# pps-lab/rofl-project-code

Measured on AMD Instinct MI355X. Metric: range-proof elements/sec (create+verify), d=25k 32-bit, higher is better.
Workload: dtype u32x8 (255-bit integer field)

## Files before the change

include/rofl_zk_debug.h:

```cpp
#ifndef ROFL_ZK_DEBUG_H
#define ROFL_ZK_DEBUG_H
#include "rofl_zk.h"
#ifdef __cplusplus
extern "C" {
#endif

typedef struct {
    double total_ms;
    double msm_accumulate_ms;
    uint64_t msm_accumulate_launches;
    uint64_t msm_terms;
    double fold_ms;
    uint64_t fold_launches;
    uint64_t fold_point_reads;
    double host_ms;
    uint64_t msm_additions;
} rofl_timing_t;
int rofl_last_timing(rofl_timing_t *out);
enum { ROFL_TK_MSM_ACCUMULATE_FB = 0, ROFL_TK_MSM_ACCUMULATE_GEN = 1, ROFL_TK_MSM_SCATTER = 2, ROFL_TK_MSM_REDUCE = 3,
       ROFL_TK_MSM_SMALL = 4, ROFL_TK_FOLD_TAB = 5, ROFL_TK_FOLD = 6, ROFL_TK_OTHER = 7,
       ROFL_TK_SIGMA = 8,
       ROFL_TK_VERIFY_SCALARS = 9,
       ROFL_TK_CODEC = 10,
       ROFL_TK_COUNT = 11 };
// ... 60 lines not shown
int rofl_dbg_rotate_tile_log2(void);
int rofl_dbg_host_dh(const uint8_t sk32[32], const uint8_t *own_pk32, const uint8_t peer_pk32[32], uint8_t out32[32], uint8_t *status);
int rofl_dbg_host_shamir_share(size_t n_secrets, const uint8_t *secrets32, const uint8_t *coef_seeds32, size_t threshold, size_t n_shares,
                               const uint32_t *xs, uint8_t *shares_out32);
int rofl_dbg_host_shamir_reconstruct(size_t n_secrets, size_t n_shares, const uint32_t *xs, const uint8_t *shares32, uint8_t *secrets_out32);
int rofl_dbg_host_feldman_commit(size_t n_secrets, const uint8_t *secrets32, const uint8_t *coef_seeds32, size_t threshold,
                                 uint8_t *commitments_out32);
int rofl_dbg_host_feldman_verify(size_t n_secrets, size_t threshold, const uint8_t *commitments32, size_t n_shares, const uint32_t *xs,
                                 const uint8_t *shares32, uint8_t *verdict_out);
int rofl_dbg_host_sig_sign(size_t n_keys, const uint8_t *sk32, uint8_t *pk_out32, size_t n_msgs, const uint8_t *msg_bytes,
                           const uint64_t *msg_off, size_t n, const rofl_sig_ref_t *refs, uint8_t *sig_out64);
int rofl_dbg_host_sig_verify(size_t n_keys, const uint8_t *pk32, size_t n_msgs, const uint8_t *msg_bytes, const uint64_t *msg_off,
                             size_t n, const rofl_sig_ref_t *refs, const uint8_t *sig64, uint8_t *verdict_out);
int rofl_dbg_host_aead_seal(size_t n_keys, const uint8_t *key32, const uint64_t *derive_round, size_t n, const uint32_t *key_idx,
                            const uint8_t *nonce12, const uint8_t *ad_bytes, const uint64_t *ad_off, const uint8_t *pt_bytes,
                            const uint64_t *pt_off, uint8_t *sealed_out);
int rofl_dbg_host_aead_open(size_t n_keys, const uint8_t *key32, const uint64_t *derive_round, size_t n, const uint32_t *key_idx,
                            const uint8_t *nonce12, const uint8_t *ad_bytes, const uint64_t *ad_off, const uint8_t *sealed_bytes,
                            const uint64_t *sealed_off, uint8_t *pt_out, uint8_t *verdict_out);
int rofl_dbg_poly1305(size_t n, const uint8_t *key32 , const uint8_t *msg_bytes, const uint64_t *msg_off ,
                      uint8_t *tag_out16 );
int rofl_dbg_host_poly1305(size_t n, const uint8_t *key32, const uint8_t *msg_bytes, const uint64_t *msg_off, uint8_t *tag_out16);
int rofl_dbg_host_dleq_prove(size_t n_own, const uint8_t *sk32, uint8_t *own_pk_out32, size_t n_peer, const uint8_t *peer_pk32, size_t n_pairs,
                             const rofl_dh_pair_t *pairs, const uint8_t *ctx32, uint8_t *reveal_out32, uint8_t *proof_out64, uint8_t *status_out);
int rofl_dbg_host_dleq_verify(size_t n_own, const uint8_t *own_pk32, size_t n_peer, const uint8_t *peer_pk32, size_t n_pairs,
                              const rofl_dh_pair_t *pairs, const uint8_t *ctx32, const uint8_t *reveal32, const uint8_t *proof64,
                              uint8_t *shared_out32, uint8_t *verdict_out);
int rofl_dbg_var_mul2(size_t n, const uint8_t *k1_32, const uint8_t *p1_32, const uint8_t *k2_32, const uint8_t *p2_32, uint8_t *out32, double *kernel_ms);
int rofl_dbg_var_mul_sum(size_t n, const uint8_t *k1_32, const uint8_t *p1_32, const uint8_t *k2_32, const uint8_t *p2_32, uint8_t *out32, double *kernel_ms);
int rofl_dbg_lane_scan(const uint8_t *needle, size_t n, int *found);

int rofl_dbg_host_bench(int what, unsigned iters, double *ns_out);
int rofl_dbg_host_horner8_selftest(unsigned W, unsigned c, int lanes, double *us_simd, double *us_scalar);
int rofl_dbg_host_encode8_selftest(unsigned batches, double *us_simd, double *us_scalar);
int rofl_dbg_host_merlin8_selftest(int lanes, unsigned count, unsigned skew, double *us_simd, double *us_scalar);
int rofl_dbg_host_merlin8_lbl3_selftest(int lanes, unsigned count, unsigned skew, double *us_simd, double *us_scalar);
int rofl_dbg_host_merlin8_lbl3_strided_selftest(int lanes, unsigned count, unsigned skew, unsigned stride, double *us_simd, double *us_scalar);
int rofl_dbg_host_merlin_run_selftest(unsigned count, unsigned skew);
int rofl_dbg_host_keccak_zmm_selftest(unsigned states, unsigned chain, double *ns_zmm, double *ns_scalar);
int rofl_dbg_last_hops(double out[10]);

#ifdef __cplusplus
}
#endif
#endif
```

rofl_project_code_amd/csrc/host51x8.hpp:

```cpp
#pragma once
#include <immintrin.h>
#include <string.h>
#include "host51.hpp"

namespace rofl {
namespace h8 {

#define ROFL_H8 __attribute__((target("avx512f,avx512ifma,avx512dq,avx512vl"))) inline

typedef __m512i V;
struct fe8 { V v[5]; };
struct ge8 { fe8 X, Y, Z, T; };

inline bool available() {
    static const bool ok = __builtin_cpu_supports("avx512f") && __builtin_cpu_supports("avx512ifma") && __builtin_cpu_supports("avx512dq");
    return ok;
}

ROFL_H8 V bc(u64 x) { return _mm512_set1_epi64((long long)x); }
ROFL_H8 void carry(fe8 &h) {
    const V M = bc(h51::M51);
    V c;
    c = _mm512_srli_epi64(h.v[0], 51); h.v[0] = _mm512_and_si512(h.v[0], M); h.v[1] = _mm512_add_epi64(h.v[1], c);
    c = _mm512_srli_epi64(h.v[1], 51); h.v[1] = _mm512_and_si512(h.v[1], M); h.v[2] = _mm512_add_epi64(h.v[2], c);
    c = _mm512_srli_epi64(h.v[2], 51); h.v[2] = _mm512_and_si512(h.v[2], M); h.v[3] = _mm512_add_epi64(h.v[3], c);
    c = _mm512_srli_epi64(h.v[3], 51); h.v[3] = _mm512_and_si512(h.v[3], M); h.v[4] = _mm512_add_epi64(h.v[4], c);
    c = _mm512_srli_epi64(h.v[4], 51); h.v[4] = _mm512_and_si512(h.v[4], M);
    V c19 = _mm512_add_epi64(_mm512_add_epi64(_mm512_slli_epi64(c, 4), _mm512_slli_epi64(c, 1)), c);
    h.v[0] = _mm512_add_epi64(h.v[0], c19);
    c = _mm512_srli_epi64(h.v[0], 51); h.v[0] = _mm512_and_si512(h.v[0], M); h.v[1] = _mm512_add_epi64(h.v[1], c);
}
ROFL_H8 fe8 add(const fe8 &a, const fe8 &b) { fe8 r; for (int i = 0; i < 5; i++) r.v[i] = _mm512_add_epi64(a.v[i], b.v[i]); carry(r); return r; }
ROFL_H8 fe8 sub(const fe8 &a, const fe8 &b) {
    fe8 r;
    r.v[0] = _mm512_sub_epi64(_mm512_add_epi64(a.v[0], bc(0x1fffffffffffb4ULL)), b.v[0]);
    for (int i = 1; i < 5; i++) r.v[i] = _mm512_sub_epi64(_mm512_add_epi64(a.v[i], bc(0x1ffffffffffffcULL)), b.v[i]);
    carry(r); return r;
}
ROFL_H8 fe8 mul(const fe8 &a, const fe8 &b) {
    const V Z = _mm512_setzero_si512();
    V lo[9], hi[9];
    for (int k = 0; k < 9; k++) { lo[k] = Z; hi[k] = Z; }
#pragma GCC unroll 5
    for (int i = 0; i < 5; i++)
#pragma GCC unroll 5
        for (int j = 0; j < 5; j++) {
            lo[i + j] = _mm512_madd52lo_epu64(lo[i + j], a.v[i], b.v[j]);
            hi[i + j] = _mm512_madd52hi_epu64(hi[i + j], a.v[i], b.v[j]);
        }
    V col[10];
    col[0] = lo[0];
    for (int c = 1; c < 9; c++) col[c] = _mm512_add_epi64(lo[c], _mm512_slli_epi64(hi[c - 1], 1));
    col[9] = _mm512_slli_epi64(hi[8], 1);
    fe8 r;
    for (int c = 0; c < 5; c++) {
        V x = col[c + 5];
        V x19 = _mm512_add_epi64(_mm512_add_epi64(_mm512_slli_epi64(x, 4), _mm512_slli_epi64(x, 1)), x);
        r.v[c] = _mm512_add_epi64(col[c], x19);
    }
    carry(r); return r;
}
ROFL_H8 fe8 sq(const fe8 &a) {
    const V Z = _mm512_setzero_si512();
    V lo[9], hi[9], xl[9], xh[9];
    for (int k = 0; k < 9; k++) { lo[k] = Z; hi[k] = Z; xl[k] = Z; xh[k] = Z; }
#pragma GCC unroll 5
    for (int i = 0; i < 5; i++) {
        lo[2 * i] = _mm512_madd52lo_epu64(lo[2 * i], a.v[i], a.v[i]);
        hi[2 * i] = _mm512_madd52hi_epu64(hi[2 * i], a.v[i], a.v[i]);
#pragma GCC unroll 5
        for (int j = i + 1; j < 5; j++) {
            xl[i + j] = _mm512_madd52lo_epu64(xl[i + j], a.v[i], a.v[j]);
            xh[i + j] = _mm512_madd52hi_epu64(xh[i + j], a.v[i], a.v[j]);
        }
    }
    V col[10];
    for (int c = 0; c < 10; c++) {
        V x = c < 9 ? _mm512_add_epi64(lo[c], _mm512_slli_epi64(xl[c], 1)) : Z;
        if (c > 0) x = _mm512_add_epi64(x, _mm512_add_epi64(_mm512_slli_epi64(hi[c - 1], 1), _mm512_slli_epi64(xh[c - 1], 2)));
        col[c] = x;
    }
    fe8 r;
    for (int c = 0; c < 5; c++) {
        V x = col[c + 5];
        V x19 = _mm512_add_epi64(_mm512_add_epi64(_mm512_slli_epi64(x, 4), _mm512_slli_epi64(x, 1)), x);
        r.v[c] = _mm512_add_epi64(col[c], x19);
    }
    carry(r); return r;
}
ROFL_H8 fe8 zero() { fe8 r; for (int i = 0; i < 5; i++) r.v[i] = _mm512_setzero_si512(); return r; }
ROFL_H8 fe8 neg(const fe8 &a) { return sub(zero(), a); }
ROFL_H8 fe8 bcast(const h51::fe5 &a) { fe8 r; for (int i = 0; i < 5; i++) r.v[i] = bc(a.v[i]); return r; }

ROFL_H8 ge8 gadd(const ge8 &p, const ge8 &q, const fe8 &d2) {
    fe8 A = mul(sub(p.Y, p.X), sub(q.Y, q.X)), B = mul(add(p.Y, p.X), add(q.Y, q.X));
    fe8 C = mul(mul(p.T, q.T), d2), D = mul(p.Z, q.Z); D = add(D, D);
    fe8 E = sub(B, A), F = sub(D, C), G = add(D, C), H = add(B, A);
    ge8 r = {mul(E, F), mul(G, H), mul(F, G), mul(E, H)};
    return r;
}
ROFL_H8 ge8 gdouble(const ge8 &p) {
    fe8 A = sq(p.X), B = sq(p.Y), C = sq(p.Z); C = add(C, C);
    fe8 E = sub(sub(sq(add(p.X, p.Y)), A), B), G = sub(B, A), F = sub(G, C), H = neg(add(A, B));
    ge8 r = {mul(E, F), mul(G, H), mul(F, G), mul(E, H)};
    return r;
}

ROFL_H8 ge8 load8(const ge *const pts[8]) {
    alignas(64) u64 t[4][5][8];
    for (int l = 0; l < 8; l++) {
        const fe *co[4] = {&pts[l]->X, &pts[l]->Y, &pts[l]->Z, &pts[l]->T};
        for (int c = 0; c < 4; c++) { h51::fe5 f = h51::from_fe_loose(*co[c]); for (int i = 0; i < 5; i++) t[c][i][l] = f.v[i]; }
    }
    ge8 r; fe8 *dst[4] = {&r.X, &r.Y, &r.Z, &r.T};
    for (int c = 0; c < 4; c++) { for (int i = 0; i < 5; i++) dst[c]->v[i] = _mm512_load_si512((const void *)t[c][i]); carry(*dst[c]); }
    return r;
}
ROFL_H8 void store8(h51::ge5 out[8], const ge8 &p) {
    alignas(64) u64 t[4][5][8];
    const fe8 *src[4] = {&p.X, &p.Y, &p.Z, &p.T};
    for (int c = 0; c < 4; c++) for (int i = 0; i < 5; i++) _mm512_store_si512((void *)t[c][i], src[c]->v[i]);
    for (int l = 0; l < 8; l++) {
        h51::fe5 *dst[4] = {&out[l].X, &out[l].Y, &out[l].Z, &out[l].T};
        for (int c = 0; c < 4; c++) for (int i = 0; i < 5; i++) dst[c]->v[i] = t[c][i][l];
    }
}

template <class GetPt>
ROFL_H8 void horner8(h51::ge5 out[8], int lanes, int W, const u32 *pos, GetPt wsum) {
    const fe8 d2 = bcast(h51::K().d2);
    const ge *p8[8];
    for (int l = 0; l < 8; l++) p8[l] = wsum(l < lanes ? l : 0, W - 1);
    ge8 acc = load8(p8);
    for (int w = W - 2; w >= 0; w--) {
        for (u32 i = pos[w]; i < pos[w + 1]; i++) acc = gdouble(acc);
        for (int l = 0; l < 8; l++) p8[l] = wsum(l < lanes ? l : 0, w);
        acc = gadd(acc, load8(p8), d2);
    }
    store8(out, acc);
}

typedef __mmask8 M8;
ROFL_H8 fe8 freeze(fe8 t) {
    const V M = bc(h51::M51);
    carry(t); carry(t);
    t.v[0] = _mm512_add_epi64(t.v[0], bc(19)); carry(t);
    t.v[0] = _mm512_add_epi64(t.v[0], bc((1ULL << 51) - 19));
    for (int i = 1; i < 5; i++) t.v[i] = _mm512_add_epi64(t.v[i], bc((1ULL << 51) - 1));
    V c;
    c = _mm512_srli_epi64(t.v[0], 51); t.v[0] = _mm512_and_si512(t.v[0], M); t.v[1] = _mm512_add_epi64(t.v[1], c);
    c = _mm512_srli_epi64(t.v[1], 51); t.v[1] = _mm512_and_si512(t.v[1], M); t.v[2] = _mm512_add_epi64(t.v[2], c);
    c = _mm512_srli_epi64(t.v[2], 51); t.v[2] = _mm512_and_si512(t.v[2], M); t.v[3] = _mm512_add_epi64(t.v[3], c);
    c = _mm512_srli_epi64(t.v[3], 51); t.v[3] = _mm512_and_si512(t.v[3], M); t.v[4] = _mm512_add_epi64(t.v[4], c);
    t.v[4] = _mm512_and_si512(t.v[4], M);
    return t;
}
ROFL_H8 M8 isneg(const fe8 &a) { fe8 c = freeze(a); return _mm512_test_epi64_mask(c.v[0], bc(1)); }
ROFL_H8 M8 iszero(const fe8 &a) {
    fe8 c = freeze(a);
    V o = _mm512_or_si512(_mm512_or_si512(c.v[0], c.v[1]), _mm512_or_si512(_mm512_or_si512(c.v[2], c.v[3]), c.v[4]));
    return _mm512_testn_epi64_mask(o, o);
}
ROFL_H8 M8 eq(const fe8 &a, const fe8 &b) { return iszero(sub(a, b)); }
ROFL_H8 fe8 blend(M8 pick_b, const fe8 &a, const fe8 &b) { fe8 r; for (int i = 0; i < 5; i++) r.v[i] = _mm512_mask_blend_epi64(pick_b, a.v[i], b.v[i]); return r; }
ROFL_H8 fe8 fabs8(const fe8 &a) { return blend(isneg(a), a, neg(a)); }
ROFL_H8 fe8 sqn(fe8 a, int n) { for (int i = 0; i < n; i++) a = sq(a); return a; }
ROFL_H8 fe8 one() { fe8 r = zero(); r.v[0] = bc(1); return r; }
ROFL_H8 fe8 pow22523(const fe8 &z) {
// ... 11 lines not shown
    M8 flipped = eq(check, neg_one), flipped_i = eq(check, mul(neg_one, sqrtm1));
    r = blend((M8)(flipped | flipped_i), r, mul(r, sqrtm1));
    return fabs8(r);
}
ROFL_H8 ge8 load8(const h51::ge5 pts[8]) {
    alignas(64) u64 t[4][5][8];
    for (int l = 0; l < 8; l++) {
        const h51::fe5 *co[4] = {&pts[l].X, &pts[l].Y, &pts[l].Z, &pts[l].T};
        for (int c = 0; c < 4; c++) for (int i = 0; i < 5; i++) t[c][i][l] = co[c]->v[i];
    }
    ge8 r; fe8 *dst[4] = {&r.X, &r.Y, &r.Z, &r.T};
    for (int c = 0; c < 4; c++) { for (int i = 0; i < 5; i++) dst[c]->v[i] = _mm512_load_si512((const void *)t[c][i]); carry(*dst[c]); }
    return r;
}
ROFL_H8 void encode8(uint8_t out[8][32], const h51::ge5 pts[8]) {
    const fe8 sqrtm1 = bcast(h51::K().sqrtm1), iamd = bcast(h51::K().invsqrt_a_minus_d);
    ge8 p = load8(pts);
    fe8 u1 = mul(add(p.Z, p.Y), sub(p.Z, p.Y)), u2 = mul(p.X, p.Y);
    fe8 is = invsqrt(mul(u1, sq(u2)), sqrtm1);
    fe8 den1 = mul(is, u1), den2 = mul(is, u2), z_inv = mul(mul(den1, den2), p.T);
    fe8 ix0 = mul(p.X, sqrtm1), iy0 = mul(p.Y, sqrtm1), ench = mul(den1, iamd);
    M8 rotate = isneg(mul(p.T, z_inv));
    fe8 x = blend(rotate, p.X, iy0), y = blend(rotate, p.Y, ix0), den_inv = blend(rotate, den2, ench);
    y = blend(isneg(mul(x, z_inv)), y, neg(y));
    fe8 s = freeze(fabs8(mul(den_inv, sub(p.Z, y))));
    alignas(64) u64 t[5][8];
    for (int i = 0; i < 5; i++) _mm512_store_si512((void *)t[i], s.v[i]);
    for (int l = 0; l < 8; l++) {
        u64 w[4] = {t[0][l] | (t[1][l] << 51), (t[1][l] >> 13) | (t[2][l] << 38), (t[2][l] >> 26) | (t[3][l] << 25), (t[3][l] >> 39) | (t[4][l] << 12)};
        memcpy(out[l], w, 32);
    }
}

}
}
```

rofl_project_code_amd/csrc/host_msm.hpp:

```cpp
#pragma once

MsmPlan msm_plan(size_t n, size_t np = 1) {
    MsmPlan p;
    static const size_t t13 = knob("ROFL_MSM_T13") ? (size_t)atol(knob("ROFL_MSM_T13")) : ((size_t)1 << 13);
    static const size_t t10_knob = knob("ROFL_MSM_T10") ? (size_t)atol(knob("ROFL_MSM_T10")) : 0;
    const size_t t10 = t10_knob ? t10_knob : (np >= 32 ? (size_t)1 << 11 : (size_t)1 << 9);
    if (n >= (1u << 17)) p.c = 16; else if (n >= t13) p.c = 13; else if (n >= t10) p.c = 10; else if (n >= 64) p.c = 7; else p.c = 4;
    if (const char *e = knob("ROFL_MSM_C")) { int v = atoi(e); if (v == 4 || v == 7 || v == 10 || v == 13 || v == 16) p.c = (u32)v; }
    p.W = (254 + p.c - 1) / p.c;
    p.W = (253 - p.c + p.c - 1) / p.c + 1;
    p.wide = (253 - p.c) - (p.c - 1) * (p.W - 1);
    p.B = 1u << (p.c - 1);
    p.levels = (p.c - 1) / 3;
    return p;
}
struct MsmOpt { u32 lr_nh = 0, lr_ng = 0; const niels *fb_wtab = nullptr; size_t fb_stride = 0; u32 fb_c = 16; std::function<void()> overlap; std::function<void(size_t)> post; u32 tag = 0;
                std::function<void(size_t, int)> post8;
                const sc *ip_dev = nullptr; u32 ip_nblk = 0; const niels *qpts = nullptr; bool *ip_included = nullptr;
                hipEvent_t pts_ready = nullptr; };

struct MsmAllow { bool fb = true, small = true, two = true, slots = true; };
enum class MsmKind { FixedBase, Small, Slots, CountSort };
struct MsmJob {
    MsmWs *ws = nullptr; size_t np = 0, nq = 0, n = 0, PW = 0; MsmPlan P{}; MsmKind kind = MsmKind::CountSort; bool lr = false, two = false, dev_horner = false;
// ... 270 lines not shown
thread_local rofl_msm_attempt_t t_msm_trace[kMsmTraceMax];
thread_local u32 t_msm_trace_n = 0;
bool msm_retry_inner(const MsmJob &J, MsmAllow &al);
bool msm_retry(const MsmJob &J, MsmAllow &al) {
    const bool small = J.kind == MsmKind::Small, two = J.two;
    const bool again = msm_retry_inner(J, al);
    g_msm_stat[again ? (small ? 1 : two ? 2 : 3) : 0].fetch_add(1, std::memory_order_relaxed);
    if (t_msm_trace_n < kMsmTraceMax)
        t_msm_trace[t_msm_trace_n++] = rofl_msm_attempt_t{
            J.fb() ? (uint32_t)ROFL_MSM_FIXED_BASE : small ? (uint32_t)ROFL_MSM_SMALL : J.kind == MsmKind::Slots ? (uint32_t)ROFL_MSM_SLOTS : (uint32_t)ROFL_MSM_COUNT_SORT,
            two ? 1u : 0u, J.P.c, J.P.W, J.cap, J.cap_bin, J.fb() ? J.sets : 0u, small ? J.small_group : 0u,
            J.host8 ? (uint32_t)ROFL_MSM_FIN_HOST8 : J.dev_horner ? (uint32_t)ROFL_MSM_FIN_DEVICE : (uint32_t)ROFL_MSM_FIN_HOST, *J.ws->h_ovf.as<u32>(4), again ? 1u : 0u};
    return again;
}
bool msm_retry_inner(const MsmJob &J, MsmAllow &al) {
    u32 flag = *J.ws->h_ovf.as<u32>(4);
    if (knob("ROFL_TRACE") && J.kind != MsmKind::CountSort)
        fprintf(stderr, "[rofl] msm np=%zu n=%zu c=%u cap=%u fb=%u lr=%d overflow=%u kind=%s two=%d bin=%u tile=%u group=%u fused_t=%u bal=%u horner=%s\n", J.np, J.n, J.P.c, J.cap, J.fb() ? J.sets : 0u, (int)J.lr, flag,
                J.fb() ? "fb" : J.kind == MsmKind::Small ? "small" : "slots", (int)J.two, J.cap_bin, J.tile, J.kind == MsmKind::Small ? J.small_group : 0u, J.fused_t, J.acc_bal, J.host8 ? "host8" : J.dev_horner ? "dev" : "host");
    if (J.kind == MsmKind::Small) { if (flag) { al.small = false; return true; } return false; }
    if (J.two) { if (flag) { al.two = false; return true; } return false; }
    if (J.kind == MsmKind::CountSort) return false;
    if (flag > MSM_OVF_MAX) { if (J.fb()) al.fb = false; else al.slots = false; return true; }
    return false;
}

void msm_finish(Ctx &C, const MsmJob &J, std::vector<ge5> &results, const MsmOpt &opt) {
    const size_t np = J.np, PW = J.PW; const MsmPlan &P = J.P; const u32 sets = J.sets;
    u32 nb = P.c - 1;
    ge *h = J.ws->h_res.as<ge>(PW * (size_t)P.c + np);
    double t0 = now_ms();
    results.resize(np);
    std::vector<double> cpu_each(np, 0.0);
    const char *fin = "host";
    if (J.host8) {
        fin = "host8";
        u32 pos[64];
        for (u32 w = 0; w < P.W; w++) pos[w] = w + 1 == P.W ? 253 - P.c : (w < P.wide ? w * P.c : P.wide * P.c + (w - P.wide) * (P.c - 1));
        C.pool->run((np + 7) / 8, [&](size_t b) {
            double tc0 = now_ms();
            size_t p0 = b * 8; int lanes = (int)std::min<size_t>(8, np - p0);
            ge5 out[8];
            h8::horner8(out, lanes, (int)P.W, pos, [&](int l, int w) { return (const ge *)&h[(p0 + (size_t)l) * P.W + (size_t)w]; });
            for (int l = 0; l < lanes; l++) results[p0 + l] = out[l];
            if (opt.post8) opt.post8(p0, lanes);
            else if (opt.post) for (int l = 0; l < lanes; l++) opt.post(p0 + l);
            cpu_each[p0] = now_ms() - tc0;
        });
    } else if (J.dev_horner) {
        fin = "dev";
        if (opt.post) C.pool->run(np, [&](size_t p) { results[p] = h51::from_ge_loose(h[p]); opt.post(p); });
        else for (size_t p = 0; p < np; p++) results[p] = h51::from_ge_loose(h[p]);
    } else if (J.fb()) {
        auto fb_one = [&](size_t p) {
            size_t base = p * sets;
            ge5 acc = h51::identity(); bool started = false;
            for (int l = (int)nb - 1; l >= 0; l--) {
                if (started) acc = h51::gdouble(acc);
                for (u32 s = 0; s < sets; s++) { acc = h51::gadd(acc, h51::from_ge_loose(h[PW + (base + s) * nb + l])); started = true; }
                if (l == 0) for (u32 s = 0; s < sets; s++) acc = h51::gadd(acc, h51::from_ge_loose(h[base + s]));
            }
            results[p] = acc;
        };
        static const size_t fb8_min = knob("ROFL_MSM_FB_HOST8_MIN") ? (size_t)std::max(1L, atol(knob("ROFL_MSM_FB_HOST8_MIN"))) : 8;
        if (opt.post8 && np >= fb8_min && h8::available() && sets * (nb + 1) <= 64) {
            fin = "fb8";
            const int Wn = (int)(sets * (nb + 1));
            u32 pos[64];
            for (u32 s = 0; s < sets; s++) pos[s] = 0;
            for (u32 l = 0; l < nb; l++) for (u32 s = 0; s < sets; s++) pos[sets + l * sets + s] = l;
            C.pool->run((np + 7) / 8, [&](size_t b) {
                double tc0 = now_ms();
                size_t p0 = b * 8; int cnt = (int)std::min<size_t>(8, np - p0);
                ge5 out[8];
                h8::horner8(out, cnt, Wn, pos, [&](int l, int w) {
                    const size_t base = (p0 + (size_t)l) * sets;
                    if ((u32)w < sets) return (const ge *)&h[base + (size_t)w];
                    const u32 lv = ((u32)w - sets) / sets, s = ((u32)w - sets) % sets;
                    return (const ge *)&h[PW + (base + s) * nb + lv];
                });
                for (int l = 0; l < cnt; l++) results[p0 + (size_t)l] = out[l];
                opt.post8(p0, cnt);
                cpu_each[p0] = now_ms() - tc0;
            });
        } else {
            fin = "fb";
            C.pool->run(np, [&](size_t p) {
                double tc0 = now_ms();
                fb_one(p); if (opt.post) opt.post(p); cpu_each[p] = now_ms() - tc0;
            });
        }
    } else {
        auto horner_range = [&](size_t p, int w_hi, int w_lo, bool down_to_zero) {
            ge5 acc = h51::identity(); bool started = false;
            for (int w = w_hi; w >= w_lo; w--) {
                size_t pw = p * P.W + w;
                int width = (u32)w + 1 == P.W ? (int)P.c + 1 : ((u32)w < P.wide ? (int)P.c : (int)P.c - 1);
                for (int l = width - 1; l >= 0; l--) {
                    if (started) acc = h51::gdouble(acc);
                    if (l <= (int)P.c - 2) { acc = h51::gadd(acc, h51::from_ge_loose(h[PW + pw * nb + l])); started = true; }
                    if (l == 0) { acc = h51::gadd(acc, h51::from_ge_loose(h[pw])); started = true; }
                }
            }
            if (down_to_zero && w_lo > 0 && started) {
                u32 pos = (u32)w_lo < P.wide ? (u32)w_lo * P.c : P.wide * P.c + ((u32)w_lo - P.wide) * (P.c - 1);
                for (u32 i = 0; i < pos; i++) acc = h51::gdouble(acc);
            }
            return acc;
        };
        const bool split = np * 2 <= 32 && P.W >= 8;
        if (split) fin = "split";
        if (!split) {
            C.pool->run(np, [&](size_t p) {
                double tc0 = now_ms();
                results[p] = horner_range(p, (int)P.W - 1, 0, false); if (opt.post) opt.post(p); cpu_each[p] = now_ms() - tc0;
            });
        } else {
            const int w_split = (int)P.W - (int)(P.W * 3 / 8);
            std::vector<ge5> part(2 * np);
            std::unique_ptr<std::atomic<int>[]> half_done(new std::atomic<int>[np]);
            for (size_t p = 0; p < np; p++) half_done[p].store(0);
            C.pool->run(2 * np, [&](size_t t) {
                double tc0 = now_ms();
                size_t p = t >> 1; bool upper = (t & 1) != 0;
                part[t] = upper ? horner_range(p, (int)P.W - 1, w_split, true) : horner_range(p, w_split - 1, 0, false);
                if (half_done[p].fetch_add(1) == 1) { results[p] = h51::gadd(part[2 * p], part[2 * p + 1]); if (opt.post) opt.post(p); }
                double dt = now_ms() - tc0; if (dt > cpu_each[p]) cpu_each[p] = dt;
            });
        }
    }
    if (knob("ROFL_TRACE")) fprintf(stderr, "[rofl] msm-finish np=%zu c=%u finish=%s\n", np, P.c, fin);
    C.tm.t.host_ms += now_ms() - t0;
    { double w = now_ms() - t0; C.hs.horner_wall += w; C.hs.max_horner = std::max(C.hs.max_horner, w); double mx = 0; for (double v : cpu_each) mx = std::max(mx, v); C.hs.horner_cpu += mx; C.hs.max_task = std::max(C.hs.max_task, mx); } C.hs.n++;
}

void msm_run(Ctx &C, const std::vector<MsmProb> &probs, size_t n, std::vector<ge5> &results, const MsmOpt &opt = MsmOpt()) {
    MsmAllow al; bool overlap_done = false;
    t_msm_trace_n = 0;
    for (;;) {
        double t_enter = now_ms();
        MsmJob J = msm_enqueue(C, C.mws[0], probs, n, opt, al);
        if (opt.overlap && !overlap_done) { opt.overlap(); overlap_done = true; }
        double t_sync0 = now_ms(); C.hs.enqueue += t_sync0 - t_enter; C.hs.max_enqueue = std::max(C.hs.max_enqueue, t_sync0 - t_enter);
        const uint64_t wkey = ((uint64_t)opt.tag << 40) ^ ((uint64_t)probs.size() << 28) ^ (uint64_t)n;
        if (opt.tag) { auto it = C.wait_ms.find(wkey); C.pool->expect_gap(it == C.wait_ms.end() ? 0.0 : it->second * 1e3); }
        C.sync();
        { double w = now_ms() - t_sync0; C.hs.sync += w; C.hs.max_sync = std::max(C.hs.max_sync, w);
          if (opt.tag) { double &e = C.wait_ms[wkey]; e = e == 0 ? w : std::min(w, 0.5 * (e + w)); } }
        if (msm_retry(J, al)) continue;
        msm_finish(C, J, results, opt);
        return;
    }
}
void msm_run2(Ctx &C, const std::vector<MsmProb> &pa, size_t na, const MsmOpt &oa, std::vector<ge5> &ra,
              const std::vector<MsmProb> &pb, size_t nb, const MsmOpt &ob, std::vector<ge5> &rb) {
    MsmAllow ala, alb;
    double t_enter = now_ms();
    if (!C.stream2) HIPCHK(hipStreamCreateWithFlags(&C.stream2, hipStreamNonBlocking));
    if (!C.ev_m2) { HIPCHK(hipEventCreateWithFlags(&C.ev_m2, hipEventDisableTiming)); HIPCHK(hipEventCreateWithFlags(&C.ev_m2j, hipEventDisableTiming)); }
    struct Join { hipStream_t s; ~Join() { (void)hipStreamSynchronize(s); } } join{C.stream2};
    HIPCHK(hipEventRecord(C.ev_m2, C.stream));
    HIPCHK(hipStreamWaitEvent(C.stream2, C.ev_m2, 0));
    MsmJob Jb = msm_enqueue(C, C.mws[1], pb, nb, ob, alb, C.stream2);
    HIPCHK(hipEventRecord(C.ev_m2j, C.stream2));
// ... 12 lines not shown
```

rofl_project_code_amd/csrc/host_rt.hpp:

```cpp
#pragma once

struct Knob { const char *name, *dflt, *what; };
static const Knob KNOBS[] = {
    {"ROFL_LANES", "3", "calls that can be in flight on a device (HIP stream + workspace each); 1..16, larger values are clamped (with a note on stderr)"},
    {"ROFL_DEVICES", "0", "option devices: bit mask of the logical devices the batch entry points shard their clients over (0 = the calling thread's device only)"},
    {"ROFL_DEVICE_MAP", "", "logical -> physical HIP device, comma separated (0,0 = two logical devices on GPU 0: how the multi-device paths are tested on a one-GPU box); default: identity"},
    {"ROFL_RCCL_LIB", "librccl.so.1", "the RCCL library rofl_comm_* loads with dlopen (a host that has torch in the process names /opt/rocm/lib/librccl.so.1: the bare soname would resolve to torch's bundled copy)"},
    {"ROFL_HOST_THREADS", "usable cores, in [2, 16]", "threads of the primary lane's host pool (window combination, encodings, transcripts of a round); other lanes: usable cores, in [6, 12]"},
    {"ROFL_POOL_SPIN_US", "400", "how long an idle pool worker polls for the next job before it sleeps (0 = sleep at once)"},
    {"ROFL_BLOCKING_SYNC", "-1", "option blocking_sync: -1 spin while <= 3 calls are in flight, 0 always spin, 1 sleep between polls"},
    {"ROFL_VERIFY_ZIP_TRUNCATE", "0", "option verify_zip_truncate: 1 = the reference's zip-truncating verify_rangeproof"},
    {"ROFL_VERIFY_BATCH", "1", "option verify_batch: 0 = one check per proof, 1 = one per client, 2 = one per batch of clients (bisecting down to per-client checks on failure)"},
    {"ROFL_SIGMA_BATCH", "1", "option sigma_batch: 0 = one check per element in the Sigma-proof verifiers"},
    {"ROFL_STAGE_KEEP_MB", "256", "pinned staging memory a lane keeps between calls (a call that needed more frees it when it ends)"},
    {"ROFL_GENS_LAZY", "1", "0 = the first call of a shape waits for its full fold table (otherwise it is served from the compact table while a background thread builds the full one)"},
    {"ROFL_GENS_LAZY_IDLE_MS", "20", "the background build of a full fold table starts when no call has been in flight for this long (its allocation stalls every HIP call of the process)"},
    {"ROFL_GENS_LAZY_MAX_WAIT_MS", "3000", "... or after this long, whichever comes first (a host that never pauses still gets its full table)"},
    {"ROFL_GENS_RESERVE_MB", "40960", "HBM a table allocation of 4 GB or more leaves free on the device (other contexts / processes / workspaces; the runtime aborts when HBM runs out): the table is narrowed instead"},
    {"ROFL_GENS_BUDGET_MB", "131072", "HBM budget of the generator-table cache (LRU eviction of unpinned entries beyond it)"},
    {"ROFL_FOLD_T1", "3", "IPP rounds before the first generator fold (1..6)"},
    {"ROFL_FOLD_T", "2", "IPP rounds between later folds (1..6)"},
    {"ROFL_FOLD_MIN", "1024", "no fold once fewer generators per chunk would remain (launches with many chunks fold down to 64)"},
    {"ROFL_MSM_BIN_SIGMA", "8", "room of a coarse bin of the two-level sort above twice its mean load, in standard deviations of that load (0 = the fixed 256 entries of rounds 2-3)"},
    {"ROFL_FOLD_TAB", "1", "0 = first fold without the precomputed odd-multiple slices"},
// ... 176 lines not shown
                            continue;
                        }
                    }
                    if (std::chrono::duration<double, std::micro>(std::chrono::steady_clock::now() - t0).count() > spin_us) break;
                }
                if (g != seen) { seen = g; my_hint = hint_seq.load(std::memory_order_acquire); work(); continue; }
            }
            for (;;) {
                asleep[my_index].store(1, std::memory_order_seq_cst);
                if (stop.load(std::memory_order_seq_cst) || gen.load(std::memory_order_seq_cst) != seen) { asleep[my_index].store(0, std::memory_order_relaxed); break; }
                syscall(SYS_futex, reinterpret_cast<uint32_t *>(&asleep[my_index]), FUTEX_WAIT_PRIVATE, 1u, nullptr, nullptr, 0);
                if (asleep[my_index].load(std::memory_order_acquire) == 0) break;
            }
            if (stop.load()) return;
            seen = gen.load(std::memory_order_acquire);
            my_hint = hint_seq.load(std::memory_order_acquire);
            work();
        }
    }
    template <class Pred> static void spin_until(Pred ready) {
        for (unsigned i = 0; !ready(); i++) {
            if (i < 20000) __builtin_ia32_pause(); else std::this_thread::yield();
        }
    }
public:
    explicit HostPool(int nthreads, const std::atomic<int> *in_flight = nullptr) : calls_in_flight(in_flight) {
        if (const char *e = knob("ROFL_POOL_SPIN_US")) spin_us = atof(e);
        asleep.reset(new std::atomic<uint32_t>[nthreads > 0 ? nthreads : 1]);
        for (int i = 0; i < nthreads; i++) asleep[i].store(0);
        for (int i = 1; i < nthreads; i++) workers.emplace_back([this, i] { loop(i); });
    }
    ~HostPool() { stop.store(true, std::memory_order_seq_cst); for (size_t w = 1; w <= workers.size(); w++) wake((int)w); for (auto &t : workers) t.join(); }
    double spin() const { return spin_us; }
    void expect_gap(double us) { gap_us.store(us, std::memory_order_relaxed); hint_seq.fetch_add(1, std::memory_order_release); }
    void run(size_t n, std::function<void(size_t)> f) {
        if (n <= 1 || workers.empty()) { for (size_t i = 0; i < n; i++) f(i); return; }
        spin_until([&] { return active.load() == 0; });
        {
            int want = (int)std::min<size_t>(n, workers.size() + 1);
            recent_max = std::max(recent_max, want);
            if (want > hot.load(std::memory_order_relaxed)) hot.store(want, std::memory_order_relaxed);
            if (++recent_runs >= 64) { hot.store(recent_max, std::memory_order_relaxed); recent_max = 0; recent_runs = 0; }
        }
        { std::lock_guard<std::mutex> lk(mu); count = 0; fn = std::move(f); done = 0; next = 0; first_error = nullptr; count = n; gen.fetch_add(1, std::memory_order_seq_cst); }
        for (size_t w = 1; w < n && w <= workers.size(); w++) wake((int)w);
        work();
        spin_until([&] { return done.load() >= n; });
        if (first_error) { std::exception_ptr e; { std::lock_guard<std::mutex> lk(err_mu); e = first_error; first_error = nullptr; } std::rethrow_exception(e); }
    }
};

struct DevBuf {
    void *p = nullptr; size_t cap = 0;
    void *ensure(size_t bytes) {
        if (bytes > cap) {
            if (p) HIPCHK(hipFree(p));
            p = nullptr; cap = 0;
            size_t want = bytes + bytes / 8 + 256;
            HIPCHK(hipMalloc(&p, want)); cap = want;
        }
        return p;
    }
    template <class T> T *as(size_t count) { return reinterpret_cast<T *>(ensure(count * sizeof(T))); }
};
struct PinBuf {
    void *p = nullptr, *dp = nullptr; size_t cap = 0;
// ... 626 lines not shown
```

rofl_project_code_amd/csrc/rofl_zk.hip:

```cpp
#include <hip/hip_runtime.h>
#include <rccl/rccl.h>
#include <dlfcn.h>
#include <immintrin.h>
#include <chrono>
#include <time.h>
#include <sched.h>
#include <unistd.h>
#include <sys/syscall.h>
#include <linux/futex.h>
#include <cmath>
#include <cstdio>
#include <cstdlib>
#include <map>
#include <memory>
#include <atomic>
#include <condition_variable>
#include <deque>
#include <exception>
#include <functional>
#include <mutex>
#include <shared_mutex>
#include <stdexcept>
#include <thread>
#include <string>
// ... 2839 lines not shown
int rofl_dbg_host_horner8_selftest(unsigned W, unsigned c, int lanes, double *us_simd, double *us_scalar) {
    if (!h8::available()) return -1;
    if (W < 2 || W > 64 || c < 2 || c > 16 || lanes < 1 || lanes > 8) return ROFL_BAD_PARAM;
    static const uint8_t Bc[32] = {0xe2, 0xf2, 0xae, 0x0a, 0x6a, 0xbc, 0x4e, 0x71, 0xa8, 0x84, 0xa9, 0x61, 0xc5, 0x00, 0x51, 0x5f,
                                   0x58, 0xe3, 0x0b, 0x6a, 0xa5, 0x82, 0xdd, 0x8d, 0xb6, 0xa6, 0x59, 0x45, 0xe0, 0x8d, 0x2d, 0x76};
    ge b; ristretto_decode(b, Bc);
    u32 pos[64]; for (unsigned w = 0; w < W; w++) pos[w] = w * c;
    std::vector<ge> pts(8 * W);
    ge5 cur = h51::from_ge(b);
    for (size_t i = 0; i < pts.size(); i++) {
        cur = h51::gadd(h51::gdouble(cur), h51::from_ge(b)); if (i % 3 == 0) cur = h51::gdouble(cur);
        pts[i] = h51::to_ge(cur);
        if (i % 4 == 1) { u64 cy = 0; const u32 pw[8] = {0xffffffedu, 0xffffffffu, 0xffffffffu, 0xffffffffu, 0xffffffffu, 0xffffffffu, 0xffffffffu, 0x7fffffffu};
                          for (int k = 0; k < 8; k++) { cy += (u64)pts[i].X.v[k] + pw[k]; pts[i].X.v[k] = (u32)cy; cy >>= 32; } }
    }
    auto wsum = [&](int l, int w) { return (const ge *)&pts[(size_t)l * W + w]; };
    uint8_t ref[8][32], got[8][32];
    double t0 = now_ms();
    for (int l = 0; l < lanes; l++) {
        ge5 acc = h51::from_ge_loose(*wsum(l, (int)W - 1));
        for (int w = (int)W - 2; w >= 0; w--) { for (u32 i = pos[w]; i < pos[w + 1]; i++) acc = h51::gdouble(acc); acc = h51::gadd(acc, h51::from_ge_loose(*wsum(l, w))); }
        h51::encode(ref[l], acc);
    }
    double t1 = now_ms();
    ge5 out[8];
    h8::horner8(out, lanes, (int)W, pos, wsum);
    double t2 = now_ms();
    int bad = 0;
    for (int l = 0; l < lanes; l++) { h51::encode(got[l], out[l]); bad |= memcmp(got[l], ref[l], 32) != 0; }
    if (us_simd) *us_simd = (t2 - t1) * 1e3;
    if (us_scalar) *us_scalar = (t1 - t0) * 1e3;
    return bad;
}
int rofl_dbg_host_encode8_selftest(unsigned batches, double *us_simd, double *us_scalar) {
    if (!h8::available()) return -1;
    static const uint8_t Bc[32] = {0xe2, 0xf2, 0xae, 0x0a, 0x6a, 0xbc, 0x4e, 0x71, 0xa8, 0x84, 0xa9, 0x61, 0xc5, 0x00, 0x51, 0x5f,
                                   0x58, 0xe3, 0x0b, 0x6a, 0xa5, 0x82, 0xdd, 0x8d, 0xb6, 0xa6, 0x59, 0x45, 0xe0, 0x8d, 0x2d, 0x76};
    ge b; ristretto_decode(b, Bc);
    ge5 b5 = h51::from_ge(b), cur = b5;
    int bad = 0; double ts = 0, tv = 0;
    for (unsigned it = 0; it < batches; it++) {
        ge5 pts[8];
        for (int l = 0; l < 8; l++) {
            cur = h51::gadd(h51::gdouble(cur), b5); if ((it + l) % 3 == 0) cur = h51::gdouble(cur);
            pts[l] = cur;
        }
        if (it == 0) { pts[0] = h51::identity(); pts[1] = b5; pts[2] = h51::gdouble(b5); pts[3] = h51::gadd(b5, h51::identity()); }
        uint8_t ref[8][32], got[8][32];
        double t0 = now_ms();
        for (int l = 0; l < 8; l++) h51::encode(ref[l], pts[l]);
        double t1 = now_ms();
        h8::encode8(got, pts);
        double t2 = now_ms();
        ts += t1 - t0; tv += t2 - t1;
        bad |= memcmp(ref, got, sizeof ref) != 0;
    }
    if (us_simd) *us_simd = tv * 1e3 / (batches ? batches : 1);
    if (us_scalar) *us_scalar = ts * 1e3 / (batches ? batches : 1);
    return bad;
}
int rofl_dbg_host_merlin_run_selftest(unsigned count, unsigned skew) {
    if (skew > 400) return ROFL_BAD_PARAM;
    std::vector<uint8_t> data((size_t)count * 32 + 1);
    for (size_t i = 0; i < data.size(); i++) data[i] = (uint8_t)((i * 2246822519u) >> 11);
    std::vector<uint8_t> pre(skew, 0xa5);
    Merlin a("RangeProof", 10), b("RangeProof", 10);
// ... 228 lines not shown
```

Before: 1.178 million.

## Add two-problem AVX-512 Horner chain packing X/Y/Z/T coordinates across lanes

Adds a horner2x4 path that packs the four coordinates of two MSM results into one 8-lane AVX-512 vector. Doubling and addition then each use one packed multiply or square via lane permutes, with a lazier carry. Small batches (np ≤ 8, or ≤ 16 when the pool has enough threads) use it instead of the 8-lane horner8, so parallelism over few problems comes from threads rather than idle SIMD lanes. It also skips computing T on intermediate doublings in horner8. The risk is extra permute and blend overhead, and loose-carry bounds that could overflow.

Result: no change. 1.192 million (median of 5 runs) (+1.2%).

```diff
diff --git a/include/rofl_zk_debug.h b/include/rofl_zk_debug.h
--- a/include/rofl_zk_debug.h
+++ b/include/rofl_zk_debug.h
@@ -116,6 +116,9 @@
 
 int rofl_dbg_host_bench(int what, unsigned iters, double *ns_out);
 int rofl_dbg_host_horner8_selftest(unsigned W, unsigned c, int lanes, double *us_simd, double *us_scalar);
+int rofl_dbg_host_horner2x4_selftest(unsigned W, unsigned c, int problems, double *us_scalar, double *us_pair);
+int rofl_dbg_host_horner_chains(int impl, unsigned threads, unsigned W, const uint32_t *pos, unsigned problems, const uint8_t *pts,
+                                uint8_t *out_xyzt, uint8_t *out_enc, double *us);
 int rofl_dbg_host_encode8_selftest(unsigned batches, double *us_simd, double *us_scalar);
 int rofl_dbg_host_merlin8_selftest(int lanes, unsigned count, unsigned skew, double *us_simd, double *us_scalar);
 int rofl_dbg_host_merlin8_lbl3_selftest(int lanes, unsigned count, unsigned skew, double *us_simd, double *us_scalar);
diff --git a/rofl_project_code_amd/csrc/host51x8.hpp b/rofl_project_code_amd/csrc/host51x8.hpp
--- a/rofl_project_code_amd/csrc/host51x8.hpp
+++ b/rofl_project_code_amd/csrc/host51x8.hpp
@@ -37,7 +37,7 @@
     for (int i = 1; i < 5; i++) r.v[i] = _mm512_sub_epi64(_mm512_add_epi64(a.v[i], bc(0x1ffffffffffffcULL)), b.v[i]);
     carry(r); return r;
 }
-ROFL_H8 fe8 mul(const fe8 &a, const fe8 &b) {
+ROFL_H8 fe8 mul_cols(const fe8 &a, const fe8 &b) {
     const V Z = _mm512_setzero_si512();
     V lo[9], hi[9];
     for (int k = 0; k < 9; k++) { lo[k] = Z; hi[k] = Z; }
@@ -58,9 +58,10 @@
         V x19 = _mm512_add_epi64(_mm512_add_epi64(_mm512_slli_epi64(x, 4), _mm512_slli_epi64(x, 1)), x);
         r.v[c] = _mm512_add_epi64(col[c], x19);
     }
-    carry(r); return r;
-}
-ROFL_H8 fe8 sq(const fe8 &a) {
+    return r;
+}
+ROFL_H8 fe8 mul(const fe8 &a, const fe8 &b) { fe8 r = mul_cols(a, b); carry(r); return r; }
+ROFL_H8 fe8 sq_cols(const fe8 &a) {
     const V Z = _mm512_setzero_si512();
     V lo[9], hi[9], xl[9], xh[9];
     for (int k = 0; k < 9; k++) { lo[k] = Z; hi[k] = Z; xl[k] = Z; xh[k] = Z; }
@@ -86,8 +87,9 @@
         V x19 = _mm512_add_epi64(_mm512_add_epi64(_mm512_slli_epi64(x, 4), _mm512_slli_epi64(x, 1)), x);
         r.v[c] = _mm512_add_epi64(col[c], x19);
     }
-    carry(r); return r;
-}
+    return r;
+}
+ROFL_H8 fe8 sq(const fe8 &a) { fe8 r = sq_cols(a); carry(r); return r; }
 ROFL_H8 fe8 zero() { fe8 r; for (int i = 0; i < 5; i++) r.v[i] = _mm512_setzero_si512(); return r; }
 ROFL_H8 fe8 neg(const fe8 &a) { return sub(zero(), a); }
 ROFL_H8 fe8 bcast(const h51::fe5 &a) { fe8 r; for (int i = 0; i < 5; i++) r.v[i] = bc(a.v[i]); return r; }
@@ -103,6 +105,12 @@
     fe8 A = sq(p.X), B = sq(p.Y), C = sq(p.Z); C = add(C, C);
     fe8 E = sub(sub(sq(add(p.X, p.Y)), A), B), G = sub(B, A), F = sub(G, C), H = neg(add(A, B));
     ge8 r = {mul(E, F), mul(G, H), mul(F, G), mul(E, H)};
+    return r;
+}
+ROFL_H8 ge8 gdouble_xyz(const ge8 &p) {
+    fe8 A = sq(p.X), B = sq(p.Y), C = sq(p.Z); C = add(C, C);
+    fe8 E = sub(sub(sq(add(p.X, p.Y)), A), B), G = sub(B, A), F = sub(G, C), H = neg(add(A, B));
+    ge8 r = {mul(E, F), mul(G, H), mul(F, G), p.T};
     return r;
 }
 
@@ -133,7 +141,7 @@
     for (int l = 0; l < 8; l++) p8[l] = wsum(l < lanes ? l : 0, W - 1);
     ge8 acc = load8(p8);
     for (int w = W - 2; w >= 0; w--) {
-        for (u32 i = pos[w]; i < pos[w + 1]; i++) acc = gdouble(acc);
+        for (u32 i = pos[w]; i < pos[w + 1]; i++) acc = i + 1 < pos[w + 1] ? gdouble_xyz(acc) : gdouble(acc);
         for (int l = 0; l < 8; l++) p8[l] = wsum(l < lanes ? l : 0, w);
         acc = gadd(acc, load8(p8), d2);
     }
@@ -211,5 +219,101 @@
     }
 }
 
-}
-}
+typedef fe8 pt2;
+#define ROFL_PERM4(a, b, c, d) ((a) | ((b) << 2) | ((c) << 4) | ((d) << 6))
+template <int IMM> ROFL_H8 fe8 perm4(const fe8 &a) { fe8 r; for (int i = 0; i < 5; i++) r.v[i] = _mm512_permutex_epi64(a.v[i], IMM); return r; }
+ROFL_H8 u64 p4_limb(int i) { return i == 0 ? 0x1fffffffffffb4ULL : 0x1ffffffffffffcULL; }
+ROFL_H8 void wcarry2(fe8 &h) {
+    const V M = bc(h51::M51);
+    V c[5];
+    for (int i = 0; i < 5; i++) { c[i] = _mm512_srli_epi64(h.v[i], 51); h.v[i] = _mm512_and_si512(h.v[i], M); }
+    V c19 = _mm512_add_epi64(_mm512_add_epi64(_mm512_slli_epi64(c[4], 4), _mm512_slli_epi64(c[4], 1)), c[4]);
+    h.v[0] = _mm512_add_epi64(h.v[0], c19);
+    for (int i = 1; i < 5; i++) h.v[i] = _mm512_add_epi64(h.v[i], c[i - 1]);
+}
+ROFL_H8 fe8 mul1(const fe8 &a, const fe8 &b) { fe8 r = mul_cols(a, b); wcarry2(r); return r; }
+ROFL_H8 fe8 sq1(const fe8 &a) { fe8 r = sq_cols(a); wcarry2(r); return r; }
+ROFL_H8 pt2 load2(const ge *p0, const ge *p1) {
+    alignas(64) u64 t[5][8];
+    const ge *pp[2] = {p0, p1};
+    for (int j = 0; j < 2; j++) {
+        const fe *co[4] = {&pp[j]->X, &pp[j]->Y, &pp[j]->Z, &pp[j]->T};
+        for (int c = 0; c < 4; c++) { h51::fe5 f = h51::from_fe_loose(*co[c]); for (int i = 0; i < 5; i++) t[i][4 * j + c] = f.v[i]; }
+    }
+    pt2 r;
+    for (int i = 0; i < 5; i++) r.v[i] = _mm512_load_si512((const void *)t[i]);
+    wcarry2(r);
+    return r;
+}
+ROFL_H8 void store2(h51::ge5 out[2], pt2 p) {
+    alignas(64) u64 t[5][8];
+    carry(p);
+    for (int i = 0; i < 5; i++) _mm512_store_si512((void *)t[i], p.v[i]);
+    for (int j = 0; j < 2; j++) {
+        h51::fe5 *dst[4] = {&out[j].X, &out[j].Y, &out[j].Z, &out[j].T};
+        for (int c = 0; c < 4; c++) for (int i = 0; i < 5; i++) dst[c]->v[i] = t[i][4 * j + c];
+    }
+}
+ROFL_H8 fe8 prep_consts() {
+    const h51::fe5 one = h51::one(), d2 = h51::K().d2;
+    fe8 r;
+    for (int i = 0; i < 5; i++) r.v[i] = _mm512_mask_blend_epi64((M8)0x44, bc(one.v[i]), bc(d2.v[i]));
+    return r;
+}
+ROFL_H8 pt2 dbl2(const pt2 &p) {
+    fe8 a = perm4<ROFL_PERM4(0, 1, 2, 0)>(p), y = perm4<ROFL_PERM4(1, 1, 1, 1)>(p);
+    for (int i = 0; i < 5; i++) a.v[i] = _mm512_mask_add_epi64(a.v[i], (M8)0x88, a.v[i], y.v[i]);
+    wcarry2(a);
+    const fe8 s = sq1(a);
+    const fe8 pa = perm4<ROFL_PERM4(0, 0, 0, 0)>(s), pb = perm4<ROFL_PERM4(1, 1, 1, 1)>(s);
+    fe8 u;
+    for (int i = 0; i < 5; i++) {
+        V t = _mm512_add_epi64(pa.v[i], _mm512_maskz_set1_epi64((M8)0xdd, (long long)p4_limb(i)));
+        t = _mm512_mask_sub_epi64(t, (M8)0x55, t, pb.v[i]);
+        t = _mm512_mask_add_epi64(t, (M8)0xaa, t, pb.v[i]);
+        t = _mm512_mask_add_epi64(t, (M8)0x44, t, _mm512_add_epi64(s.v[i], s.v[i]));
+        u.v[i] = _mm512_mask_sub_epi64(t, (M8)0x88, t, s.v[i]);
+    }
+    wcarry2(u);
+    return mul1(perm4<ROFL_PERM4(3, 0, 2, 3)>(u), perm4<ROFL_PERM4(2, 1, 0, 1)>(u));
+}
+ROFL_H8 fe8 ymx_ypx(const pt2 &p, bool twice_z) {
+    const fe8 a = perm4<ROFL_PERM4(1, 1, 3, 2)>(p), b = perm4<ROFL_PERM4(0, 0, 2, 2)>(p);
+    const M8 plus = twice_z ? (M8)0xaa : (M8)0x22;
+    fe8 r;
+    for (int i = 0; i < 5; i++) {
+        V t = _mm512_add_epi64(a.v[i], _mm512_maskz_set1_epi64((M8)0x11, (long long)p4_limb(i)));
+        t = _mm512_mask_sub_epi64(t, (M8)0x11, t, b.v[i]);
+        r.v[i] = _mm512_mask_add_epi64(t, plus, t, b.v[i]);
+    }
+    wcarry2(r);
+    return r;
+}
+ROFL_H8 pt2 prep2(const pt2 &q, const fe8 &consts) { return mul1(ymx_ypx(q, true), consts); }
+ROFL_H8 pt2 add2(const pt2 &p, const pt2 &q_prepared) {
+    const fe8 m = mul1(ymx_ypx(p, false), q_prepared);
+    const fe8 p1 = perm4<ROFL_PERM4(1, 3, 3, 1)>(m), p2 = perm4<ROFL_PERM4(0, 2, 2, 0)>(m);
+    fe8 u;
+    for (int i = 0; i < 5; i++) {
+        V t = _mm512_add_epi64(p1.v[i], _mm512_maskz_set1_epi64((M8)0x33, (long long)p4_limb(i)));
+        t = _mm512_mask_sub_epi64(t, (M8)0x33, t, p2.v[i]);
+        u.v[i] = _mm512_mask_add_epi64(t, (M8)0xcc, t, p2.v[i]);
+    }
+    wcarry2(u);
+    return mul1(perm4<ROFL_PERM4(0, 2, 1, 0)>(u), perm4<ROFL_PERM4(1, 3, 2, 3)>(u));
+}
+template <class GetPt>
+ROFL_H8 void horner2x4(h51::ge5 out[2], int count, int W, const u32 *pos, GetPt wsum) {
+    const fe8 consts = prep_consts();
+    const int l1 = count > 1 ? 1 : 0;
+    pt2 acc = load2(wsum(0, W - 1), wsum(l1, W - 1));
+    for (int w = W - 2; w >= 0; w--) {
+        const pt2 q = prep2(load2(wsum(0, w), wsum(l1, w)), consts);
+        for (u32 i = pos[w]; i < pos[w + 1]; i++) acc = dbl2(acc);
+        acc = add2(acc, q);
+    }
+    store2(out, acc);
+}
+
+}
+}
diff --git a/rofl_project_code_amd/csrc/host_msm.hpp b/rofl_project_code_amd/csrc/host_msm.hpp
--- a/rofl_project_code_amd/csrc/host_msm.hpp
+++ b/rofl_project_code_amd/csrc/host_msm.hpp
@@ -326,12 +326,28 @@
     double t0 = now_ms();
     results.resize(np);
     std::vector<double> cpu_each(np, 0.0);
-    const char *fin = "host";
+    const char *fin = "host", *chain = nullptr;
+    constexpr size_t kPairMax = 16;
+    const bool pair = np <= 8 || (np <= kPairMax && np <= 2 * C.pool->threads());
+    auto pair_post = [&](size_t p0, int cnt) {
+        if (opt.post8) opt.post8(p0, cnt);
+        else if (opt.post) for (int l = 0; l < cnt; l++) opt.post(p0 + (size_t)l);
+    };
     if (J.host8) {
         fin = "host8";
         u32 pos[64];
         for (u32 w = 0; w < P.W; w++) pos[w] = w + 1 == P.W ? 253 - P.c : (w < P.wide ? w * P.c : P.wide * P.c + (w - P.wide) * (P.c - 1));
-        C.pool->run((np + 7) / 8, [&](size_t b) {
+        chain = pair ? "pair" : "lane";
+        if (pair) C.pool->run((np + 1) / 2, [&](size_t b) {
+            double tc0 = now_ms();
+            size_t p0 = b * 2; int cnt = (int)std::min<size_t>(2, np - p0);
+            ge5 out[2];
+            h8::horner2x4(out, cnt, (int)P.W, pos, [&](int l, int w) { return (const ge *)&h[(p0 + (size_t)l) * P.W + (size_t)w]; });
+            for (int l = 0; l < cnt; l++) results[p0 + (size_t)l] = out[l];
+            pair_post(p0, cnt);
+            cpu_each[p0] = now_ms() - tc0;
+        });
+        else C.pool->run((np + 7) / 8, [&](size_t b) {
             double tc0 = now_ms();
             size_t p0 = b * 8; int lanes = (int)std::min<size_t>(8, np - p0);
             ge5 out[8];
@@ -363,16 +379,27 @@
             u32 pos[64];
             for (u32 s = 0; s < sets; s++) pos[s] = 0;
             for (u32 l = 0; l < nb; l++) for (u32 s = 0; s < sets; s++) pos[sets + l * sets + s] = l;
-            C.pool->run((np + 7) / 8, [&](size_t b) {
+            auto fb_wsum = [&](size_t p, int w) {
+                const size_t base = p * sets;
+                if ((u32)w < sets) return (const ge *)&h[base + (size_t)w];
+                const u32 lv = ((u32)w - sets) / sets, s = ((u32)w - sets) % sets;
+                return (const ge *)&h[PW + (base + s) * nb + lv];
+            };
+            chain = pair ? "pair" : "lane";
+            if (pair) C.pool->run((np + 1) / 2, [&](size_t b) {
+                double tc0 = now_ms();
+                size_t p0 = b * 2; int cnt = (int)std::min<size_t>(2, np - p0);
+                ge5 out[2];
+                h8::horner2x4(out, cnt, Wn, pos, [&](int l, int w) { return fb_wsum(p0 + (size_t)l, w); });
+                for (int l = 0; l < cnt; l++) results[p0 + (size_t)l] = out[l];
+                opt.post8(p0, cnt);
+                cpu_each[p0] = now_ms() - tc0;
+            });
+            else C.pool->run((np + 7) / 8, [&](size_t b) {
                 double tc0 = now_ms();
                 size_t p0 = b * 8; int cnt = (int)std::min<size_t>(8, np - p0);
                 ge5 out[8];
-                h8::horner8(out, cnt, Wn, pos, [&](int l, int w) {
-                    const size_t base = (p0 + (size_t)l) * sets;
-                    if ((u32)w < sets) return (const ge *)&h[base + (size_t)w];
-                    const u32 lv = ((u32)w - sets) / sets, s = ((u32)w - sets) % sets;
-                    return (const ge *)&h[PW + (base + s) * nb + lv];
-                });
+                h8::horner8(out, cnt, Wn, pos, [&](int l, int w) { return fb_wsum(p0 + (size_t)l, w); });
                 for (int l = 0; l < cnt; l++) results[p0 + (size_t)l] = out[l];
                 opt.post8(p0, cnt);
                 cpu_each[p0] = now_ms() - tc0;
@@ -423,7 +450,10 @@
             });
         }
     }
-    if (knob("ROFL_TRACE")) fprintf(stderr, "[rofl] msm-finish np=%zu c=%u finish=%s\n", np, P.c, fin);
+    if (knob("ROFL_TRACE")) {
+        if (chain) fprintf(stderr, "[rofl] msm-finish np=%zu c=%u finish=%s chain=%s\n", np, P.c, fin, chain);
+        else fprintf(stderr, "[rofl] msm-finish np=%zu c=%u finish=%s\n", np, P.c, fin);
+    }
     C.tm.t.host_ms += now_ms() - t0;
     { double w = now_ms() - t0; C.hs.horner_wall += w; C.hs.max_horner = std::max(C.hs.max_horner, w); double mx = 0; for (double v : cpu_each) mx = std::max(mx, v); C.hs.horner_cpu += mx; C.hs.max_task = std::max(C.hs.max_task, mx); } C.hs.n++;
 }
diff --git a/rofl_project_code_amd/csrc/host_rt.hpp b/rofl_project_code_amd/csrc/host_rt.hpp
--- a/rofl_project_code_amd/csrc/host_rt.hpp
+++ b/rofl_project_code_amd/csrc/host_rt.hpp
@@ -232,6 +232,7 @@
     }
     ~HostPool() { stop.store(true, std::memory_order_seq_cst); for (size_t w = 1; w <= workers.size(); w++) wake((int)w); for (auto &t : workers) t.join(); }
     double spin() const { return spin_us; }
+    size_t threads() const { return workers.size() + 1; }
     void expect_gap(double us) { gap_us.store(us, std::memory_order_relaxed); hint_seq.fetch_add(1, std::memory_order_release); }
     void run(size_t n, std::function<void(size_t)> f) {
         if (n <= 1 || workers.empty()) { for (size_t i = 0; i < n; i++) f(i); return; }
diff --git a/rofl_project_code_amd/csrc/rofl_zk.hip b/rofl_project_code_amd/csrc/rofl_zk.hip
--- a/rofl_project_code_amd/csrc/rofl_zk.hip
+++ b/rofl_project_code_amd/csrc/rofl_zk.hip
@@ -2895,6 +2895,74 @@
     if (us_scalar) *us_scalar = (t1 - t0) * 1e3;
     return bad;
 }
+int rofl_dbg_host_horner_chains(int impl, unsigned threads, unsigned W, const uint32_t *pos, unsigned problems, const uint8_t *pts_bytes,
+                                uint8_t *out_xyzt, uint8_t *out_enc, double *us) {
+    if (impl < 0 || impl > 3 || !pos || !pts_bytes || W < 1 || W > 64 || problems < 1 || problems > 4096 || pos[0] != 0) return ROFL_BAD_PARAM;
+    for (unsigned w = 1; w < W; w++) if (pos[w] < pos[w - 1] || pos[w] > 256) return ROFL_BAD_PARAM;
+    if (impl == 3 && (threads < 1 || threads > 64)) return ROFL_BAD_PARAM;
+    if (impl != 0 && !h8::available()) return -1;
+    static_assert(sizeof(ge) == 128, "a ge record is X | Y | Z | T of 32 bytes");
+    std::vector<ge> pts((size_t)problems * W);
+    memcpy(pts.data(), pts_bytes, pts.size() * sizeof(ge));
+    std::vector<ge5> res(problems);
+    auto at = [&](size_t p, int w) { return (const ge *)&pts[p * W + (size_t)w]; };
+    auto pair_task = [&](size_t b) {
+        size_t p0 = b * 2; int cnt = (int)std::min<size_t>(2, problems - p0);
+        ge5 out[2];
+        h8::horner2x4(out, cnt, (int)W, pos, [&](int l, int w) { return at(p0 + (size_t)l, w); });
+        for (int l = 0; l < cnt; l++) res[p0 + (size_t)l] = out[l];
+    };
+    std::unique_ptr<HostPool> pool;
+    if (impl == 3) { pool.reset(new HostPool((int)threads)); pool->run((problems + 1) / 2, pair_task); }
+    double t0 = now_ms();
+    if (impl == 0) {
+        for (size_t p = 0; p < problems; p++) {
+            ge5 acc = h51::from_ge_loose(*at(p, (int)W - 1));
+            for (int w = (int)W - 2; w >= 0; w--) { for (u32 i = pos[w]; i < pos[w + 1]; i++) acc = h51::gdouble(acc); acc = h51::gadd(acc, h51::from_ge_loose(*at(p, w))); }
+            res[p] = acc;
+        }
+    } else if (impl == 1) {
+        for (size_t p0 = 0; p0 < problems; p0 += 8) {
+            int lanes = (int)std::min<size_t>(8, problems - p0);
+            ge5 out[8];
+            h8::horner8(out, lanes, (int)W, pos, [&](int l, int w) { return at(p0 + (size_t)l, w); });
+            for (int l = 0; l < lanes; l++) res[p0 + (size_t)l] = out[l];
+        }
+    } else if (impl == 2) {
+        for (size_t b = 0; b < (problems + 1) / 2; b++) pair_task(b);
+    } else
+        pool->run((problems + 1) / 2, pair_task);
+    if (us) *us = (now_ms() - t0) * 1e3;
+    for (size_t p = 0; p < problems; p++) {
+        if (out_xyzt) { ge g = h51::to_ge(res[p]); memcpy(out_xyzt + p * 128, &g, 128); }
+        if (out_enc) h51::encode(out_enc + p * 32, res[p]);
+    }
+    return ROFL_OK;
+}
+int rofl_dbg_host_horner2x4_selftest(unsigned W, unsigned c, int problems, double *us_scalar, double *us_pair) {
+    if (!h8::available()) return -1;
+    if (W < 2 || W > 64 || c > 16 || c == 1 || (c == 0 && (W & 1)) || problems < 1 || problems > 2) return ROFL_BAD_PARAM;
+    static const uint8_t Bc[32] = {0xe2, 0xf2, 0xae, 0x0a, 0x6a, 0xbc, 0x4e, 0x71, 0xa8, 0x84, 0xa9, 0x61, 0xc5, 0x00, 0x51, 0x5f,
+                                   0x58, 0xe3, 0x0b, 0x6a, 0xa5, 0x82, 0xdd, 0x8d, 0xb6, 0xa6, 0x59, 0x45, 0xe0, 0x8d, 0x2d, 0x76};
+    ge b; ristretto_decode(b, Bc);
+    u32 pos[64]; for (unsigned w = 0; w < W; w++) pos[w] = c ? w * c : (w < 2 ? 0 : (w - 2) / 2);
+    std::vector<ge> pts(2 * W);
+    ge5 cur = h51::from_ge(b);
+    for (size_t i = 0; i < pts.size(); i++) {
+        cur = h51::gadd(h51::gdouble(cur), h51::from_ge(b)); if (i % 3 == 0) cur = h51::gdouble(cur);
+        pts[i] = h51::to_ge(cur);
+        if (i % 4 == 1) { u64 cy = 0; const u32 pw[8] = {0xffffffedu, 0xffffffffu, 0xffffffffu, 0xffffffffu, 0xffffffffu, 0xffffffffu, 0xffffffffu, 0x7fffffffu};
+                          for (int k = 0; k < 8; k++) { cy += (u64)pts[i].X.v[k] + pw[k]; pts[i].X.v[k] = (u32)cy; cy >>= 32; } }
+    }
+    uint8_t ref[2][32], got[2][32];
+    double us[2] = {0, 0};
+    int rc = rofl_dbg_host_horner_chains(0, 0, W, pos, (unsigned)problems, (const uint8_t *)pts.data(), nullptr, &ref[0][0], &us[0]);
+    if (rc == ROFL_OK) rc = rofl_dbg_host_horner_chains(2, 0, W, pos, (unsigned)problems, (const uint8_t *)pts.data(), nullptr, &got[0][0], &us[1]);
+    if (rc != ROFL_OK) return rc;
+    if (us_scalar) *us_scalar = us[0];
+    if (us_pair) *us_pair = us[1];
+    return memcmp(ref, got, (size_t)problems * 32) != 0;
+}
 int rofl_dbg_host_encode8_selftest(unsigned batches, double *us_simd, double *us_scalar) {
     if (!h8::available()) return -1;
     static const uint8_t Bc[32] = {0xe2, 0xf2, 0xae, 0x0a, 0x6a, 0xbc, 0x4e, 0x71, 0xa8, 0x84, 0xa9, 0x61, 0xc5, 0x00, 0x51, 0x5f,
```
